# huttered40/capital

Measured on AMD Instinct MI355X. Metric: TFLOP/s (whole node) Cholesky n=65536, algorithmic n^3/3, recursive cholinv factor(), inputs resident in HBM, higher is better.
Workload: dtype f64

## Files before the change

### capital_amd/capi.py

```python
import ctypes as C
import os

import numpy as np
import torch

_HERE = os.path.dirname(os.path.abspath(__file__))
LIB_PATH = os.environ.get("CAPITAL_HIP_LIB", os.path.join(_HERE, "libcapital_hip.so"))

NOTRANS, TRANS = 0, 1
LEFT, RIGHT = 0, 1
LOWER, UPPER = 0, 1
NONUNIT, UNIT = 0, 1
RECT, UPPERTRI, LOWERTRI = 0, 1, 2

_i64, _dbl, _int, _vp = C.c_int64, C.c_double, C.c_int, C.c_void_p

_SIGS = {
    "capi_dgemm": [_int, _int, _i64, _i64, _i64, _dbl, _vp, _i64, _vp, _i64, _dbl, _vp, _i64],
    "capi_dsyrk": [_int, _int, _i64, _i64, _dbl, _vp, _i64, _dbl, _vp, _i64],
    "capi_dgemmt": [_int, _int, _int, _i64, _i64, _dbl, _vp, _i64, _vp, _i64, _dbl, _vp, _i64],
    "capi_dsyrk_panel32": [_i64, _i64, _dbl, _vp, _dbl, _vp, _i64],
    "capi_dtrmm_right_panel32": [_i64, _i64, _dbl, _vp, _i64, _vp, _i64, _vp, _i64],
    "capi_dtrmm": [_int, _int, _int, _int, _i64, _i64, _dbl, _vp, _i64, _vp, _i64],
    "capi_dtrmm_oop": [_int, _int, _int, _int, _i64, _i64, _dbl, _vp, _i64, _vp, _i64, _vp, _i64],
    "capi_dtrmm_acc": [_int, _int, _int, _int, _i64, _i64, _dbl, _vp, _i64, _vp, _i64, _dbl, _vp, _i64],
    "capi_dtrsm": [_int, _int, _int, _int, _i64, _i64, _dbl, _vp, _i64, _vp, _i64],
    "capi_dpotrf": [_int, _i64, _vp, _i64],
    "capi_dtrtri": [_int, _int, _i64, _vp, _i64],
    "capi_dpotrf_trtri": [_i64, _vp, _i64, _vp, _i64],
    "capi_dgram_equilibrate_shift": [_i64, _vp, _i64, _i64, _dbl, _vp, _vp],
    "capi_dtri_rescale": [_i64, _vp, _i64, _vp, _i64, _vp, _vp],
    "capi_dgemtn_ts": [_i64, _i64, _i64, _dbl, _vp, _i64, _vp, _i64, _dbl, _vp, _i64],
    "capi_dresid_ts": [_i64, _i64, _i64, _vp, _i64, _vp, _i64, _vp, _i64, _vp, _i64, _vp],
    "capi_dtrmm_thin": [_int, _int, _i64, _i64, _i64, _dbl, _vp, _i64, _i64, _vp, _i64, _dbl, _vp, _i64],
    "capi_get_info": [C.POINTER(_int)],
    "capi_reset_info": [],
    "capi_serialize": [_int, _int, _vp, _i64, _i64, _vp, _i64, _i64] + [_i64] * 8,
    "capi_serialize_shape": [_int, _int, _int, _vp, _i64, _i64, _vp, _i64, _i64] + [_i64] * 8,
    "capi_dlacpy": [_int, _i64, _i64, _vp, _i64, _vp, _i64],
    "capi_dgeadd": [_int, _i64, _i64, _dbl, _vp, _i64, _dbl, _vp, _i64],
    "capi_dtrizero": [_int, _i64, _vp, _i64],
    "capi_daxpby": [_i64, _dbl, _vp, _vp],
    "capi_remove_triangle": [C.c_char, _vp, _i64, _i64, _i64, _i64, _i64],
    "capi_block_to_cyclic": [_vp, _vp, _i64, _i64, _i64],
    "capi_block_to_cyclic_full": [_vp, _vp, _i64, _i64, _i64],
    "capi_cyclic_to_block": [_vp, _vp, _i64, _i64, _i64],
    "capi_block_to_cyclic_tri": [_vp, _vp, _i64, _i64],
# ... 161 lines not shown
```

### capital_amd/csrc/gemm_f64.hip

```cpp
#include "capi_internal.h"
#include "gemm_plan.h"
#include <type_traits>

extern "C" int capi_internal_copy2d(capi_handle_t h, int64_t m, int64_t n, const double* A, int64_t lda, double* B, int64_t ldb);

typedef double d4_t __attribute__((ext_vector_type(4)));
typedef double d2_t __attribute__((ext_vector_type(2)));

namespace {

constexpr int NTHREADS = 256;
using gemm_plan::BK, gemm_plan::SK;
template <int TS> struct tile_cfg {
  static constexpr int TILE_LDS = TS * SK;
  static constexpr int STAGE_LDS = 2 * TILE_LDS;
  static constexpr int NQ = TS / 32;
  static constexpr int SUB = TS / 32;
};
constexpr int GROUP_M = 8;
template <int TS> __device__ __forceinline__ int rc_r(int tid, int q) { return 16 * ((tid >> 6) * (TS / 64) + (q >> 1)) + 2 * (tid & 7); }
__device__ __forceinline__ int rc_k(int tid, int q) { return 8 * (q & 1) + ((tid >> 3) & 7); }

struct GemmArgs {
  const double* A;
// ... 4 lines not shown
  double alpha, beta;
  int out_uplo;
  int tri_side;
  int tri_eff_upper;
  int tri_unit;
  int a_vec, b_vec;
  int splitk, k_per_split;
  int k_rotate;
  double* slab;
  int64_t slab_ld, slab_stride;
  int tiles_m, tiles_n, ntiles;
  int batch;
  int64_t sa, sb, sc;
  int tail_base, tail_tm, tail_tn;
  int ts;
  int no_skip;
  int share_ab;
  int tri_dense;
  int tri_koff;
  int tri_block;
  int pid_base;
  int order;
  int a_tiled, c_tiled;
  unsigned long long* stamp;
};

__device__ __forceinline__ void stamp_begin(const GemmArgs& p) {
  if (p.stamp && threadIdx.x == 0) atomicMin(p.stamp, (unsigned long long)wall_clock64());
}
__device__ __forceinline__ void stamp_end(const GemmArgs& p) {
  if (p.stamp && threadIdx.x == 0) atomicMin(p.stamp + 1, ~(unsigned long long)wall_clock64());
}

template <int TS, bool KC>
__device__ __forceinline__ void panel_load(const double* __restrict__ X, int64_t ld, int r0, int R, int k0, int kend,
                                           int tid, bool vec_ok, d2_t (&v)[TS / 32]) {
  constexpr int NQ = TS / 32;
  if (KC) {
    const int kp = tid & 7, rb = tid >> 3;
    const int k = k0 + 2 * kp;
#pragma unroll
    for (int q = 0; q < NQ; ++q) {
      const int r = r0 + rb + 32 * q;
      d2_t val = {0.0, 0.0};
      if (r < R) {
        const double* p = X + (int64_t)r * ld + k;
// ... 349 lines not shown
      fa += (int64_t)(t - t_in) * ksa;
      fb += (int64_t)(t - t_in) * ksb;
    }
  }

  auto element_ok = [&](int i, int j) {
    bool ok = (i < p.M) && (j < p.N);
    if (p.out_uplo == CAPI_UPPER) ok = ok && (i <= j);
    if (p.out_uplo == CAPI_LOWER) ok = ok && (i >= j);
    return ok;
  };
  if (p.splitk > 1) {
#pragma unroll
    for (int a = 0; a < SUB; ++a) {
      const int i = i0 + wm * (TS / 2) + a * 16 + r16;
#pragma unroll
      for (int b = 0; b < SUB; ++b)
#pragma unroll
        for (int reg = 0; reg < 4; ++reg) {
          const int j = j0 + wn * (TS / 2) + b * 16 + g + 4 * reg;
          if (element_ok(i, j)) p.slab[(int64_t)z * p.slab_stride + i + (int64_t)j * p.slab_ld] = acc[a][b][reg];
        }
    }
  } else if (p.beta == 0.0) {
#pragma unroll
    for (int a = 0; a < SUB; ++a) {
      const int i = i0 + wm * (TS / 2) + a * 16 + r16;
#pragma unroll
      for (int b = 0; b < SUB; ++b)
#pragma unroll
        for (int reg = 0; reg < 4; ++reg) {
          const int j = j0 + wn * (TS / 2) + b * 16 + g + 4 * reg;
          if (element_ok(i, j)) p.C[i + (int64_t)j * p.ldc] = p.alpha * acc[a][b][reg];
        }
    }
  } else {
#pragma unroll
    for (int a = 0; a < SUB; ++a) {
      const int i = i0 + wm * (TS / 2) + a * 16 + r16;
      double old[SUB][4];
#pragma unroll
      for (int b = 0; b < SUB; ++b)
#pragma unroll
        for (int reg = 0; reg < 4; ++reg) {
          const int j = j0 + wn * (TS / 2) + b * 16 + g + 4 * reg;
          const bool ok = element_ok(i, j);
// ... 154 lines not shown
        panel_store<TS, AK>(Na, tid, ra);
        panel_store<TS, BKC>(Na + TILE_LDS, tid, rb);
      }
      par ^= 1;
      __syncthreads();
    };
    auto fast_run = [&](int tc) -> int {
      if (asc) return tc < tb0 ? max(0, min(tb0, ntk) - 1 - tc) : (tc >= tb1 ? max(0, ntk - 1 - tc) : 0);
      return tc >= tb1 ? tc - tb1 : (tc < tb0 ? tc : 0);
    };
    while (t >= 0 && t < ntk) {
      const int nf = fast_run(t);
      fa = fa0 + (int64_t)t * ksa;
      fb = fb0 + (int64_t)t * ksb;
      for (int q = 0; q < nf; ++q, t += dir) iterate(t, t + dir, std::true_type{});
      while (t >= 0 && t < ntk) {
        const int tn = t + dir;
        iterate(t, (tn >= 0 && tn < ntk) ? tn : -1, std::false_type{});
        t = tn;
        if (t >= 0 && t < ntk && fast_run(t) > 0) break;
      }
    }

#pragma unroll
    for (int a = 0; a < SUB; ++a) {
      const int i = i0 + wm * (TS / 2) + a * 16 + r16;
#pragma unroll
      for (int c = 0; c < SUB; ++c)
#pragma unroll
        for (int reg = 0; reg < 4; ++reg) {
          const int j = j0 + wn * (TS / 2) + c * 16 + g + 4 * reg;
          p.C[i + (int64_t)j * p.ldc] = p.alpha * acc[a][c][reg];
        }
    }
  }
  stamp_end(p);
}

__global__ void splitk_reduce_kernel(const double* __restrict__ slab, int64_t slab_ld, int64_t slab_stride, int splitk,
                                     double* __restrict__ C, int64_t ldc, int M, int N, double alpha, double beta, int out_uplo) {
  const int i = blockIdx.x * blockDim.x + threadIdx.x;
  if (i >= M) return;
  for (int j = blockIdx.y; j < N; j += gridDim.y) {
    if (out_uplo == CAPI_UPPER && i > j) continue;
    if (out_uplo == CAPI_LOWER && i < j) continue;
    double s = 0.0;
// ... 490 lines not shown
}

__global__ __launch_bounds__(TSK_THREADS, 1) void trmm_right_ts32_kernel(const GemmArgs p) {
  extern __shared__ __attribute__((aligned(16))) double lds[];
  switch (__builtin_amdgcn_readfirstlane(threadIdx.x >> 6)) {
    case 0: trmm_ts32_body<0>(p, lds); break;
    case 1: trmm_ts32_body<1>(p, lds); break;
    case 2: trmm_ts32_body<2>(p, lds); break;
    case 3: trmm_ts32_body<3>(p, lds); break;
    case 4: trmm_ts32_body<4>(p, lds); break;
    case 5: trmm_ts32_body<5>(p, lds); break;
    case 6: trmm_ts32_body<6>(p, lds); break;
    default: trmm_ts32_body<7>(p, lds); break;
  }
}

template <int TS>
gemm_kernel_t pick_kernel(bool ak, bool bkc) {
  return ak ? (bkc ? dgemm_tile_kernel<TS, true, true> : dgemm_tile_kernel<TS, true, false>)
            : (bkc ? dgemm_tile_kernel<TS, false, true> : dgemm_tile_kernel<TS, false, false>);
}

struct GemmEnv {
  bool debug;
  int no_skip;
  gemm_plan::Overrides ov;
};
const GemmEnv& gemm_env() {
  static const GemmEnv e = [] {
    const char* fts = getenv("CAPI_FORCE_TS");
    const char* fsm = getenv("CAPI_SMALL");
    return GemmEnv{getenv("CAPI_DEBUG_GEMM") != nullptr, getenv("CAPI_NO_SKIP") ? 1 : 0, {fts ? atoi(fts) : 0, fsm ? (atoi(fsm) != 0) : -1}};
  }();
  return e;
}

int launch_recorded(capi_handle_t h, gemm_kernel_t k, int64_t grid, size_t lds_bytes, GemmArgs q, double share, int variant) {
  capi_handle_s::prof_rec* rec = nullptr;
  if (h->prof_on) {
    if (h->prof_n == h->prof_cap) {
      const int ncap = h->prof_cap ? h->prof_cap * 2 : 1024;
      auto* np_ = (capi_handle_s::prof_rec*)realloc(h->prof, sizeof(capi_handle_s::prof_rec) * ncap);
      if (!np_) return CAPI_ENOMEM;
      for (int i = h->prof_cap; i < ncap; ++i) { np_[i].e0 = nullptr; np_[i].e1 = nullptr; }
      h->prof = np_;
      h->prof_cap = ncap;
    }
    rec = &h->prof[h->prof_n++];
    if (!rec->e0) { CAPI_HIP_CHECK(h, hipEventCreate(&rec->e0)); CAPI_HIP_CHECK(h, hipEventCreate(&rec->e1)); }
    rec->flops = q.out_uplo >= 0 ? (double)q.N * ((double)q.N + 1.0) * (double)q.K
                 : (q.tri_side >= 0 ? (q.tri_block ? (double)q.M * (double)q.N * (2.0 * (double)q.tri_koff + (double)q.N) : (double)q.M * (double)q.N * (double)q.K)
                                    : 2.0 * (double)q.M * (double)q.N * (double)q.K);
    rec->flops *= share;
    rec->variant = variant;
    rec->m = q.M; rec->n = q.N; rec->k = q.K; rec->kind = q.out_uplo >= 0 ? 1 : (q.tri_side >= 0 ? 2 : 0);
// ... 12 lines not shown
    hipLaunchKernelGGL(splitk_reduce_wide_kernel, dim3((unsigned)cdiv(p.M, 64), (unsigned)p.N), dim3(256), 0, h->stream, p.slab, p.slab_ld,
                       p.slab_stride, p.splitk, p.C, p.ldc, p.M, p.N, p.alpha, p.beta, p.out_uplo);
  else
    hipLaunchKernelGGL(splitk_reduce_kernel, dim3((unsigned)cdiv(p.M, 256), (unsigned)(p.N < 65535 ? p.N : 65535)), dim3(256), 0, h->stream,
                       p.slab, p.slab_ld, p.slab_stride, p.splitk, p.C, p.ldc, p.M, p.N, p.alpha, p.beta, p.out_uplo);
  CAPI_HIP_CHECK(h, hipGetLastError());
  return CAPI_OK;
}

int launch_gemm(capi_handle_t h, bool ak, bool bkc, GemmArgs& p, bool ws_for_slab) {
  using gemm_plan::Path;
  const GemmEnv& env = gemm_env();
  gemm_plan::Product d;
  d.M = p.M; d.N = p.N; d.K = p.K; d.out_uplo = p.out_uplo;
  d.tri_side = p.tri_side; d.tri_eff_upper = p.tri_eff_upper; d.tri_dense = p.tri_dense; d.tri_block = p.tri_block; d.tri_koff = p.tri_koff;
  d.alpha_zero = p.alpha == 0.0; d.beta = p.beta; d.batch = p.batch; d.ak = ak; d.bkc = bkc;
  d.a_is_b = p.A == p.B; d.same_ld = p.lda == p.ldb;
  d.a_vec = (((uintptr_t)p.A & 15) == 0) && ((p.lda & 1) == 0);
  d.b_vec = (((uintptr_t)p.B & 15) == 0) && ((p.ldb & 1) == 0);
  d.a_tiled = p.a_tiled; d.c_tiled = p.c_tiled; d.ws_for_slab = ws_for_slab;
  const gemm_plan::Device dev{h->num_cu, h->cu_of[h->cur]};
  const gemm_plan::Modes modes{h->rounds_mode, h->pair_mode, h->pair_rounds, h->pair_rounds_min};
  const gemm_plan::Plan pl = gemm_plan::plan(d, dev, modes, env.ov);
  if (env.debug) {
    char line[2048];
    gemm_plan::format(line, sizeof(line), d, dev, modes, env.ov, pl);
    fprintf(stderr, "[capi gemm] %s\n", line);
  }
  hipStream_t s = h->stream;
  if (pl.path == Path::none) return CAPI_OK;
  CAPI_REQUIRE(h, pl.path != Path::refused, "panel32 operand reached a kernel that does not read it");
  if (pl.path == Path::scale) {
    dim3 grid((unsigned)cdiv(p.M, 256), (unsigned)(p.N < 65535 ? p.N : 65535));
    hipLaunchKernelGGL(scale_kernel, grid, dim3(256), 0, s, p.C, p.ldc, p.M, p.N, p.beta, p.out_uplo);
    CAPI_HIP_CHECK(h, hipGetLastError());
    return CAPI_OK;
  }
  if (pl.path == Path::trmm_ts32) {
    p.a_vec = d.a_vec;
    p.splitk = 1;
    CAPI_RAISE_LDS_LIMIT(h, CAPI_ATTR_TRMM_TS32, trmm_right_ts32_kernel, pl.lds_bytes);
    hipLaunchKernelGGL(trmm_right_ts32_kernel, dim3((unsigned)pl.blocks), dim3(TSK_THREADS), pl.lds_bytes, s, p);
    CAPI_HIP_CHECK(h, hipGetLastError());
    return CAPI_OK;
  }
  if (pl.path == Path::gram_blocks) {
    for (int J = 0; J < pl.tiles_n; ++J)
      for (int I = 0; I <= J; ++I) {
        GemmArgs q = p;
        q.A = p.A + (int64_t)I * TSK_W * p.lda;
// ... 124 lines not shown
  CAPI_REQUIRE(h, n >= 0 && k >= 0 && n < (1LL << 31) && k < (1LL << 31), "dims");
  if (n == 0) return CAPI_OK;
  CAPI_REQUIRE(h, C && ldc >= n, "C/ldc");
  if (k > 0) {
    CAPI_REQUIRE(h, A && B, "null operand");
    CAPI_REQUIRE(h, lda >= (transA ? k : n) && ldb >= (transB ? n : k), "lda/ldb");
  }
  GemmArgs p{};
  p.A = A; p.B = B; p.C = C; p.lda = lda; p.ldb = ldb; p.ldc = ldc;
  p.M = (int)n; p.N = (int)n; p.K = (int)k; p.alpha = alpha; p.beta = beta;
  p.out_uplo = uplo; p.tri_side = -1;
  return launch_gemm(h, transA == CAPI_TRANS, transB == CAPI_NOTRANS, p, true);
}

int capi_dsyrk(capi_handle_t h, int uplo, int trans, int64_t n, int64_t k, double alpha,
               const double* A, int64_t lda, double beta, double* C, int64_t ldc) {
  CAPI_REQUIRE(h, h, "null handle");
  CAPI_REQUIRE(h, ok01(trans), "transpose code");
  return capi_dgemmt(h, uplo, trans, trans == CAPI_TRANS ? CAPI_NOTRANS : CAPI_TRANS, n, k, alpha, A, lda, A, lda, beta, C, ldc);
}

static int trmm_launch(capi_handle_t h, int side, int uplo, int trans, int diag, int64_t m, int64_t n, double alpha,
                       const double* T, int64_t ldt, const double* B, int64_t ldb, double beta, double* C, int64_t ldc,
                       bool ws_free = true) {
  CAPI_REQUIRE(h, h, "null handle");
  CAPI_REQUIRE(h, ok01(side) && ok01(uplo) && ok01(trans) && ok01(diag), "enum code");
  CAPI_REQUIRE(h, m >= 0 && n >= 0 && m < (1LL << 31) && n < (1LL << 31), "dims");
  if (m == 0 || n == 0) return CAPI_OK;
  const int64_t nt = side == CAPI_LEFT ? m : n;
  CAPI_REQUIRE(h, T && B && C && ldt >= nt && ldb >= m && ldc >= m, "operands");
  CAPI_REQUIRE(h, (const double*)C != B, "out-of-place trmm: C aliases B");
  GemmArgs p{};
  p.C = C; p.ldc = ldc; p.M = (int)m; p.N = (int)n; p.K = (int)nt; p.alpha = alpha; p.beta = beta;
  p.out_uplo = -1;
  p.tri_side = side;
  p.tri_eff_upper = ((uplo == CAPI_UPPER) != (trans == CAPI_TRANS));
  p.tri_unit = diag == CAPI_UNIT;
  if (side == CAPI_RIGHT && diag == CAPI_NONUNIT && n >= 512 && n <= 4096 && m >= 64 * n) {
    void* w;
    int rc = capi_ws3_get(h, sizeof(double) * (size_t)n * (size_t)n, &w);
    if (rc != CAPI_OK) return rc;
    CAPI_HIP_CHECK(h, hipMemsetAsync(w, 0, sizeof(double) * (size_t)n * (size_t)n, h->stream));
    rc = capi_dlacpy(h, uplo == CAPI_UPPER ? 1 : 2, n, n, T, ldt, (double*)w, n);
    if (rc != CAPI_OK) return rc;
    T = (const double*)w;
    ldt = n;
    p.tri_dense = 1;
    const bool eff_upper = (uplo == CAPI_UPPER) != (trans == CAPI_TRANS);
    if (eff_upper && n % 256 == 0) {
      for (int64_t J = 0; J < n / 256; ++J) {
        GemmArgs q = p;
        q.N = 256;
        q.K = (int)(256 * (J + 1));
        q.tri_koff = (int)(256 * J);
        q.tri_block = 1;
        q.C = C + 256 * J * ldc;
        q.A = B; q.lda = ldb;
        q.B = trans == CAPI_NOTRANS ? T + 256 * J * ldt : T + 256 * J;
        q.ldb = ldt;
        int rc2 = launch_gemm(h, false, trans == CAPI_NOTRANS, q, ws_free);
        if (rc2 != CAPI_OK) return rc2;
      }
      return CAPI_OK;
    }
  }
  if (side == CAPI_LEFT) {
    p.A = T; p.lda = ldt; p.B = B; p.ldb = ldb;
    return launch_gemm(h, trans == CAPI_TRANS, true, p, ws_free);
  } else {
    p.A = B; p.lda = ldb; p.B = T; p.ldb = ldt;
    return launch_gemm(h, false, trans == CAPI_NOTRANS, p, ws_free);
  }
}

__attribute__((visibility("hidden"))) int capi_internal_trmm_oop_batched(capi_handle_t h, int side, int uplo, int trans, int diag,
                                                                           int64_t m, int64_t n, double alpha, const double* T,
                                                                           int64_t ldt, int64_t st, const double* B, int64_t ldb,
                                                                           int64_t sb_, double* C, int64_t ldc, int64_t sc_, int batch) {
  CAPI_REQUIRE(h, h && m >= 0 && n >= 0 && m < (1LL << 31) && n < (1LL << 31) && batch >= 0, "dims");
  const bool small_ok = m <= 512 && n <= 512 && gemm_env().ov.force_small < 0;
  const bool aligned = ((st | sb_ | sc_) & 1) == 0;
  if (batch > 1 && small_ok && aligned) {
    const int64_t nt = side == CAPI_LEFT ? m : n;
    GemmArgs p{};
    p.C = C; p.ldc = ldc; p.M = (int)m; p.N = (int)n; p.K = (int)nt; p.alpha = alpha; p.beta = 0.0;
    p.out_uplo = -1; p.tri_side = side;
    p.tri_eff_upper = ((uplo == CAPI_UPPER) != (trans == CAPI_TRANS));
    p.tri_unit = diag == CAPI_UNIT;
    p.batch = batch;
    if (side == CAPI_LEFT) { p.A = T; p.lda = ldt; p.sa = st; p.B = B; p.ldb = ldb; p.sb = sb_; p.sc = sc_; return launch_gemm(h, trans == CAPI_TRANS, true, p, true); }
    p.A = B; p.lda = ldb; p.sa = sb_; p.B = T; p.ldb = ldt; p.sb = st; p.sc = sc_;
    return launch_gemm(h, false, trans == CAPI_NOTRANS, p, true);
  }
  for (int b = 0; b < batch; ++b) {
    int rc = capi_dtrmm_oop(h, side, uplo, trans, diag, m, n, alpha, T + b * st, ldt, B + b * sb_, ldb, C + b * sc_, ldc);
    if (rc != CAPI_OK) return rc;
  }
  return CAPI_OK;
}

int capi_dtrmm_oop(capi_handle_t h, int side, int uplo, int trans, int diag, int64_t m, int64_t n, double alpha,
                   const double* T, int64_t ldt, const double* B, int64_t ldb, double* C, int64_t ldc) {
  return trmm_launch(h, side, uplo, trans, diag, m, n, alpha, T, ldt, B, ldb, 0.0, C, ldc);
}

int capi_dtrmm_acc(capi_handle_t h, int side, int uplo, int trans, int diag, int64_t m, int64_t n, double alpha,
                   const double* T, int64_t ldt, const double* B, int64_t ldb, double beta, double* C, int64_t ldc) {
  return trmm_launch(h, side, uplo, trans, diag, m, n, alpha, T, ldt, B, ldb, beta, C, ldc);
}

int capi_dtrmm(capi_handle_t h, int side, int uplo, int trans, int diag, int64_t m, int64_t n, double alpha,
               const double* T, int64_t ldt, double* B, int64_t ldb) {
  CAPI_REQUIRE(h, h, "null handle");
  if (m <= 0 || n <= 0) return m < 0 || n < 0 ? CAPI_EINVAL : CAPI_OK;
  void* ws;
  int rc = capi_ws_get(h, sizeof(double) * (size_t)m * (size_t)n, &ws);
  if (rc != CAPI_OK) return rc;
  rc = trmm_launch(h, side, uplo, trans, diag, m, n, alpha, T, ldt, B, ldb, 0.0, (double*)ws, m, false);
  if (rc != CAPI_OK) return rc;
  return capi_internal_copy2d(h, m, n, (const double*)ws, m, B, ldb);
}

int capi_dsyrk_panel32(capi_handle_t h, int64_t n, int64_t k, double alpha, const double* A32, double beta, double* C, int64_t ldc) {
  CAPI_REQUIRE(h, h, "null handle");
  CAPI_REQUIRE(h, n == TSK_W && k > 0 && k % 32 == 0 && k >= 64 * n && k < (1LL << 31), "panel32 Gram matrix: n == 256, k a multiple of 32, k >= 64 n");
  CAPI_REQUIRE(h, A32 && C && ldc >= n && (((uintptr_t)A32 & 15) == 0), "operands");
// ... 129 lines not shown
```

### capital_amd/csrc/gemm_plan.h

```cpp
#ifndef CAPITAL_GEMM_PLAN_H_
#define CAPITAL_GEMM_PLAN_H_

#include <cstddef>
#include <cstdint>
#include <cstdio>

#include "capital_hip.h"

namespace gemm_plan {

constexpr int BK = 16;
constexpr int SK = BK + 2;
constexpr int ST = 32, SKC = 256, SQK = 64, SLD = ST + 2;
constexpr int TSK_W = 256;

inline int64_t cdiv(int64_t a, int64_t b) { return (a + b - 1) / b; }

struct Product {
  int M = 0, N = 0, K = 0;
  int out_uplo = -1;
  int tri_side = -1;
  int tri_eff_upper = 0, tri_dense = 0, tri_block = 0, tri_koff = 0;
  bool alpha_zero = false;
  double beta = 0.0;
// ... 170 lines not shown
    if (r.ntiles >= 2 * per_round && rem > 0 && rem <= (3 * per_round) / 4) r.tail128 = rem;
  }
  const int ntiles_all = r.ntiles;
  r.ntiles -= r.tail128;
  r.blocks = (int64_t)r.ntiles * r.splitk;
  r.per_launch = use_rounds ? per_round : r.blocks;
  r.lds_bytes = sizeof(double) * 2 * 2 * (size_t)r.ts * SK;
  r.variant = vi + (r.ts == 128 ? 0 : 4);
  r.share_den = (double)ntiles_all * r.splitk;
  const int ntri = p.tri_side == CAPI_LEFT ? r.tiles_m : r.tiles_n, nfree = p.tri_side == CAPI_LEFT ? r.tiles_n : r.tiles_m;
  const int64_t wgs = (int64_t)(ntri / 2) * nfree;
  if (mode.pair_mode && tri && !p.tri_dense && !p.tri_block && p.tri_koff == 0 && r.ts == 128 && r.splitk == 1 && p.beta == 0.0 &&
      p.batch <= 1 && p.M % 128 == 0 && p.N % 128 == 0 && p.K % 128 == 0 && p.a_vec && p.b_vec && (ntri & 1) == 0 && wgs % per_round == 0 &&
      (mode.pair_mode > 1 || wgs <= 4 * per_round || (mode.pair_rounds && p.K >= mode.pair_rounds_min))) {
    r.path = Path::pair;
    r.blocks = wgs;
    r.per_launch = mode.pair_rounds && wgs > per_round && p.K >= mode.pair_rounds_min ? per_round : wgs;
    r.variant = vi + 16;
    r.share_den = (double)wgs;
  }
  return r;
}

inline int format(char* buf, size_t n, const Product& p, const Device& d, const Modes& m, const Overrides& o, const Plan& r) {
  static const char* const reduce_names[] = {"none", "narrow", "wide"};
  return snprintf(buf, n,
                  "M=%d N=%d K=%d out_uplo=%d tri_side=%d tri_eff_upper=%d tri_dense=%d tri_block=%d tri_koff=%d alpha_zero=%d beta=%.17g "
                  "batch=%d ak=%d bkc=%d a_is_b=%d same_ld=%d a_vec=%d b_vec=%d a_tiled=%d c_tiled=%d ws_for_slab=%d num_cu=%d stream_cu=%d "
                  "rounds_mode=%d pair_mode=%d pair_rounds=%d pair_rounds_min=%d force_ts=%d force_small=%d -> path=%s ts=%d splitk=%d "
                  "k_per_split=%d k_rotate=%d order=%d share_ab=%d slab_stride=%lld tiles_m=%d tiles_n=%d ntiles=%d blocks=%lld "
                  "per_launch=%lld launches=%lld grid_y=%d tail128=%d reduce=%s lds=%zu variant=%d share_den=%.17g est_us=%.1f small_est_us=%.1f",
                  p.M, p.N, p.K, p.out_uplo, p.tri_side, p.tri_eff_upper, p.tri_dense, p.tri_block, p.tri_koff, (int)p.alpha_zero, p.beta,
                  p.batch, (int)p.ak, (int)p.bkc, (int)p.a_is_b, (int)p.same_ld, (int)p.a_vec, (int)p.b_vec, (int)p.a_tiled, (int)p.c_tiled,
                  (int)p.ws_for_slab, d.num_cu, d.stream_cu, m.rounds_mode, m.pair_mode, m.pair_rounds, m.pair_rounds_min, o.force_ts,
                  o.force_small, path_name(r.path), r.ts, r.splitk, r.k_per_split, r.k_rotate, r.order, r.share_ab, (long long)r.slab_stride,
                  r.tiles_m, r.tiles_n, r.ntiles, (long long)r.blocks, (long long)r.per_launch, (long long)r.launches(), r.grid_y, r.tail128,
                  reduce_names[(int)r.reduce], r.lds_bytes, r.variant, r.share_den, r.est_us, r.small_est_us);
}

}

#endif
```

### capital_amd/src/alg/cholesky/cholinv/cholinv.h

```cpp
#ifndef CAPITAL_CHOLESKY_CHOLINV_H_
#define CAPITAL_CHOLESKY_CHOLINV_H_

#include "./../../alg.h"
#include "./../../matmult/summa/summa.h"
#include "./policy.h"

#pragma weak capi_dtrmm_thin
#pragma weak capi_dresid_ts

namespace cholesky {

template <class SerializePolicy = policy::cholinv::Serialize, class IntermediatesPolicy = policy::cholinv::SaveIntermediates,
          class BaseCasePolicy = policy::cholinv::NoReplication>
class cholinv : public SerializePolicy, public IntermediatesPolicy, public BaseCasePolicy {
public:
  using SP = SerializePolicy;
  using IP = IntermediatesPolicy;
  using BP = BaseCasePolicy;

  template <typename ScalarT, typename DimensionT>
  class info {
  public:
    using ScalarType = ScalarT;
    using DimensionType = DimensionT;
    using alg_type = cholinv<SerializePolicy, IntermediatesPolicy, BaseCasePolicy>;
    using SP = SerializePolicy;
    using IP = IntermediatesPolicy;
    using BP = BaseCasePolicy;
    info(const info& p) : complete_inv(p.complete_inv), split(p.split), bc_mult_dim(p.bc_mult_dim), dir(p.dir) {}
    info(info&& p) : complete_inv(p.complete_inv), split(p.split), bc_mult_dim(p.bc_mult_dim), dir(p.dir) {}
    info(DimensionType complete_inv, DimensionType split, DimensionType bc_mult_dim, char dir)
        : complete_inv(complete_inv), split(split), bc_mult_dim(bc_mult_dim), dir(dir) {}
    const DimensionType complete_inv, split, bc_mult_dim;
    const char dir;
    matrix<ScalarType, DimensionType, typename SerializePolicy::structure> R, Rinv;
    matrix<ScalarType, DimensionType, rect> Rfull, Rinvfull;
    matmult::arena work;
    DimensionType localDimension = 0, globalDimension = 0, trueLocalDimension = 0, trueGlobalDimension = 0, bcDimension = 0;
    int64_t num_base_cases = 0, num_levels = 0;
    bool solve_with_trsm = false;
    int potrf_info = 0;
    bool zeroed = false;
    const double* input = nullptr;
    DimensionType early_split = 0;
    DimensionType input_lead = 0;
    int la_depth = 0;
    bool factored = false, factored_trsm = false;
    DimensionType top_split = 0;
    matrix<ScalarType, DimensionType, rect> X, SolveW1, SolveW2, SolveRho, SolveD, SolveNorm2;
    std::vector<double> solve_residual_norms;
  };

  template <typename MatrixType, typename ArgType, typename CommType>
  static void factor(const MatrixType& A, ArgType& args, CommType&& CommInfo) {
    CRITTER_START(CI::factor);
    using U = typename ArgType::DimensionType;
    static_assert(std::is_same<typename MatrixType::StructureType, rect>::value, "cholinv::factor takes a rect-structured input block");
    if (!(args.split > 0) || args.dir != 'U') throw std::invalid_argument("cholinv: split > 0 and dir == 'U' required (cholinv.hpp:9)");
    if (CommInfo.d > 1 && CommInfo.d % CommInfo.c) throw std::invalid_argument("cholinv: c must divide d (or d == 1)");
    args.factored = false;
    args.factored_trsm = args.solve_with_trsm;
    args.top_split = 0;
    if (args.solve_with_trsm) { factor_trsm(A, args, CommInfo); args.factored = true; CRITTER_STOP(CI::factor); return; }
    const U localDimension = A.num_rows_local(), globalDimension = A.num_rows_global();
    CAPITAL_CHECK(capi_stream_select(capital::handle(), 0));
    CAPITAL_CHECK(capi_reset_info(capital::handle()));
    args.potrf_info = 0;
    args.R._register_(A.num_columns_global(), A.num_rows_global(), CommInfo.d, CommInfo.d);
    args.Rinv._register_(A.num_columns_global(), A.num_rows_global(), CommInfo.d, CommInfo.d);
    constexpr bool packed = !std::is_same<typename SP::structure, rect>::value;
    if (packed) {
      args.Rfull._register_(A.num_columns_global(), A.num_rows_global(), CommInfo.d, CommInfo.d);
      args.Rinvfull._register_(A.num_columns_global(), A.num_rows_global(), CommInfo.d, CommInfo.d);
    }
    double* R = packed ? args.Rfull.data() : (double*)args.R.data();
    double* Ri = packed ? args.Rinvfull.data() : (double*)args.Rinv.data();
    const U ld = localDimension;
    if (!args.zeroed) {
      capital::dev_zero(R, ld * ld);
      capital::dev_zero(Ri, ld * ld);
      args.zeroed = true;
    }
    U bcDimLocal = (U)(CommInfo.c * CommInfo.d);
    U bcMult = args.bc_mult_dim;
    if (bcMult < 0) { bcMult = -bcMult; for (U i = 0; i < bcMult; ++i) bcDimLocal *= 2; } else { for (U i = 0; i < bcMult; ++i) bcDimLocal /= 2; }
    bcDimLocal = std::max<U>(1, bcDimLocal);
    bcDimLocal = std::min<U>(localDimension, bcDimLocal);
    bcDimLocal = localDimension / bcDimLocal;
    args.localDimension = args.trueLocalDimension = localDimension;
    args.globalDimension = args.trueGlobalDimension = globalDimension;
    args.bcDimension = (U)CommInfo.d * bcDimLocal;
    args.num_base_cases = args.num_levels = 0;

    const U h1 = localDimension >> args.split;
    args.input = A.data();
    args.early_split = 0;
    const bool will_split = !(((localDimension * (U)CommInfo.d) <= args.bcDimension) || (h1 < args.split));
    args.input_lead = 0;
    args.top_split = will_split ? h1 : 0;
    if (will_split && h1 > 0 && h1 < ld) {
      capi_handle_t hh = capital::handle();
      U lead = h1;
      if (args.split == 1 && CommInfo.d == 1 && CommInfo.c == 1) while (lead >= 8192 && lead % 2 == 0 && (lead >> 1) * (U)CommInfo.d > args.bcDimension) lead >>= 1;
      CAPITAL_CHECK(capi_dlacpy(hh, 1, lead, lead, A.data(), ld, R, ld));
      CAPITAL_CHECK(capi_event_record(hh, EV_INPUT_HEAD));
      CAPITAL_CHECK(capi_stream_select(hh, 1));
      CAPITAL_CHECK(capi_event_wait(hh, EV_INPUT_HEAD));
      if (lead < h1) {
        CAPITAL_CHECK(capi_dlacpy(hh, 0, lead, h1 - lead, A.data() + (int64_t)lead * ld, ld, R + (int64_t)lead * ld, ld));
        CAPITAL_CHECK(capi_dlacpy(hh, 1, h1 - lead, h1 - lead, A.data() + lead + (int64_t)lead * ld, ld, R + lead + (int64_t)lead * ld, ld));
        CAPITAL_CHECK(capi_event_record(hh, EV_INPUT_MID));
        args.input_lead = lead;
      }
      CAPITAL_CHECK(capi_dlacpy(hh, 0, h1, ld - h1, A.data() + (int64_t)h1 * ld, ld, R + (int64_t)h1 * ld, ld));
      CAPITAL_CHECK(capi_dlacpy(hh, 1, ld - h1, ld - h1, A.data() + h1 + (int64_t)h1 * ld, ld, R + h1 + (int64_t)h1 * ld, ld));
      CAPITAL_CHECK(capi_event_record(hh, EV_INPUT_REST));
      CAPITAL_CHECK(capi_stream_select(hh, 0));
      args.early_split = h1;
    } else {
      CAPITAL_CHECK(capi_dlacpy(capital::handle(), 1, ld, ld, A.data(), ld, R, ld));
    }


    const bool single = (CommInfo.d == 1 && CommInfo.c == 1);
    capital::launch_rounds_scope rounds(true);
    const U h = localDimension - (localDimension >> args.split);
    const U agg = args.bcDimension;
    int64_t need = single ? (int64_t)h * h + (int64_t)h * h / 3 + 1024 : (int64_t)(CommInfo.d == 1 ? 8 : 12) * h * h + 4 * (int64_t)agg * agg + 4096;
    args.work.reserve(need);

    args.la_depth = 0;
    invoke(args, CommInfo, R, Ri, ld, (U)0, localDimension, globalDimension);

    if (packed) {
      const U e = args.early_split;
      if (e > 0) {
        pack_block(args, CAPI_UPPERTRI, R, (double*)args.R.data(), ld, e, ld, e, ld);
        pack_block(args, CAPI_UPPERTRI, Ri, (double*)args.Rinv.data(), ld, e, ld, e, ld);
        if (args.complete_inv) pack_block(args, CAPI_RECT, Ri, (double*)args.Rinv.data(), ld, e, ld, 0, e);
        CAPITAL_CHECK(capi_event_wait(capital::handle(), EV_EARLY_PACK));
      } else {
        serialize<uppertri, uppertri>::invoke(args.Rfull, args.R, 0, ld, 0, ld, 0, ld, 0, ld);
        serialize<uppertri, uppertri>::invoke(args.Rinvfull, args.Rinv, 0, ld, 0, ld, 0, ld, 0, ld);
      }
    }
    if (!IP::keep_arena) {
      capital::sync();
      args.work.release();
      if (packed) { args.Rfull._destroy_(); args.Rinvfull._destroy_(); args.zeroed = false; }
    }
    CRITTER_STOP(CI::factor);
    CAPITAL_CHECK(capi_get_info(capital::handle(), &args.potrf_info));
    const int failed = capital::ranks_with_nonzero(CommInfo.world, args.potrf_info);
    if (failed != 0)
      throw std::domain_error("cholinv::factor: the matrix is not positive definite (" +
                              (args.potrf_info != 0 ? "non-positive pivot " + std::to_string(args.potrf_info) + " of a diagonal block"
                                                    : std::string("reported by ") + std::to_string(failed) + " other rank(s) of the grid") +
// ... 273 lines not shown
      CRITTER_STOP(CI::factor_diag);
      return;
    }
    ++args.num_levels;
    const U split2 = localDim - split1;
    const bool single = (t.d == 1 && t.c == 1);
    matmult::arena& ws = args.work;
    view R11i{Ri + start + start * ld, ld, split1, split1};
    view A12{R + start + (start + split1) * ld, ld, split1, split2};
    view A22{R + (start + split1) + (start + split1) * ld, ld, split2, split2};
    view R22i{Ri + (start + split1) + (start + split1) * ld, ld, split2, split2};
    view I12{Ri + start + (start + split1) * ld, ld, split1, split2};

    invoke(args, t, R, Ri, ld, start, split1, globalDim >> 1);
    if (wait_ev >= 0) CAPITAL_CHECK(capi_event_wait(h, wait_ev));
    if (start == 0 && args.input_lead > 0 && split1 == args.input_lead) CAPITAL_CHECK(capi_event_wait(h, EV_INPUT_MID));

    const bool top = (localDim == args.localDimension) && args.early_split == split1;
    if (top) CAPITAL_CHECK(capi_event_wait(h, EV_INPUT_REST));
    CRITTER_START(CI::trsm);
    int child_wait = -1;
    bool copy_deferred = false;
    const int64_t mark = ws.top;
    {
      view W{ws.take((int64_t)split1 * split2), split1, split1, split2};
      if (single) {
        CAPITAL_CHECK(capi_dtrmm_oop(h, CAPI_LEFT, CAPI_UPPER, CAPI_TRANS, CAPI_NONUNIT, split1, split2, 1.0, R11i.p, ld, A12.p, ld, W.p, W.ld));
      } else {
        view Tx{ws.take((int64_t)split1 * split1), split1, split1, split1};
        const int64_t np = matmult::summa::tri_count(split1);
        if ((t.x == t.y && !t.multipath) || !matmult::summa::packed_comm()) {
          CAPITAL_CHECK(capi_dlacpy(h, 0, split1, split1, R11i.p, ld, Tx.p, Tx.ld));
          util::transpose_raw(Tx.p, Tx.count(), ws.take(Tx.count()), t, matmult::summa::relay_space(t, Tx.count(), ws));
        } else if (t.x == t.y) {
          CAPITAL_CHECK(capi_dlacpy(h, 0, split1, split1, R11i.p, ld, Tx.p, Tx.ld));
          util::transpose_raw(nullptr, np, nullptr, t, matmult::summa::relay_space(t, np, ws));
        } else {
          double* pk = ws.take(np);
          matmult::summa::pack_tri(R11i, CAPI_UPPER, pk);
          util::transpose_raw(pk, np, ws.take(np), t, matmult::summa::relay_space(t, np, ws));
          matmult::summa::unpack_tri(pk, CAPI_UPPER, Tx);
        }
        matmult::summa::trmm(t, CAPI_LEFT, CAPI_UPPER, CAPI_TRANS, CAPI_NONUNIT, 1.0, Tx, A12, W, ws);
      }
      const U lead = split2 >> args.split;
      const bool a22_splits = !(((split2 * (U)t.d) <= args.bcDimension) || (lead < args.split));
      const bool la = single && a22_splits && lead > 0 && lookahead_min() >= 0 && (int64_t)split2 >= lookahead_min() && args.la_depth < lookahead_depth();
      const bool pack_now = top && !std::is_same<typename SP::structure, rect>::value;
      const bool copy_later = la && pack_now && !getenv("CAPITAL_PACK_AT_ONCE");
      if (!copy_later) CAPITAL_CHECK(capi_dlacpy(h, 0, split1, split2, W.p, W.ld, A12.p, ld));
      copy_deferred = copy_later;
      CRITTER_STOP(CI::trsm);
      auto early_pack = [&](int after_ev) {
        CAPITAL_CHECK(capi_stream_select(h, 1));
        CAPITAL_CHECK(capi_event_wait(h, after_ev));
        if (copy_later) CAPITAL_CHECK(capi_dlacpy(h, 0, split1, split2, W.p, W.ld, A12.p, ld));
        pack_block(args, CAPI_UPPERTRI, R, (double*)args.R.data(), ld, (U)0, split1, (U)0, split1);
        pack_block(args, CAPI_RECT, R, (double*)args.R.data(), ld, split1, ld, (U)0, split1);
        pack_block(args, CAPI_UPPERTRI, Ri, (double*)args.Rinv.data(), ld, (U)0, split1, (U)0, split1);
        CAPITAL_CHECK(capi_event_record(h, EV_EARLY_PACK));
        CAPITAL_CHECK(capi_stream_select(h, 0));
      };
      bool packed_early = false;

      CRITTER_START(CI::tmu);
      if (la) {
        const int depth = args.la_depth;
        const U rest = split2 - lead;
        double* Wr = W.p + (int64_t)lead * W.ld;
        CAPITAL_CHECK(capi_dgemmt(h, CAPI_UPPER, CAPI_TRANS, CAPI_NOTRANS, lead, split1, -1.0, W.p, W.ld, W.p, W.ld, 1.0, A22.p, ld));
        CAPITAL_CHECK(capi_event_record(h, EV_LA_LEAD + depth));
        CAPITAL_CHECK(capi_stream_select(h, LA_STREAM0 + depth));
        CAPITAL_CHECK(capi_event_wait(h, EV_LA_LEAD + depth));
// ... 10 lines not shown
      } else {
        view Wx{ws.take(W.count()), split1, split1, split2};
        capital::dev_copy(Wx.p, W.p, W.count());
        util::transpose_raw(Wx.p, Wx.count(), ws.take(Wx.count()), t, matmult::summa::relay_space(t, Wx.count(), ws));
        matmult::summa::syrk(t, CAPI_UPPER, CAPI_TRANS, -1.0, W, Wx, 1.0, A22, ws);
      }
      if (pack_now && !packed_early) {
        CAPITAL_CHECK(capi_event_record(h, EV_TOP_R12));
        early_pack(EV_TOP_R12);
      }
      if (child_wait < 0) ws.top = mark;
      CRITTER_STOP(CI::tmu);
    }

    invoke(args, t, R, Ri, ld, start + split1, split2, split2 * (U)t.d, child_wait);
    if (child_wait >= 0) { --args.la_depth; ws.top = mark; }

    CRITTER_START(CI::tmu);
    if (!(!args.complete_inv && (globalDim == args.trueGlobalDimension))) {
      if (copy_deferred) CAPITAL_CHECK(capi_event_wait(h, EV_EARLY_PACK));
      const int64_t mark = ws.top;
      view W2{ws.take((int64_t)split1 * split2), split1, split1, split2};
      matmult::summa::trmm(t, CAPI_LEFT, CAPI_UPPER, CAPI_NOTRANS, CAPI_NONUNIT, 1.0, R11i, A12, W2, ws);
      if (single) {
        matmult::summa::trmm(t, CAPI_RIGHT, CAPI_UPPER, CAPI_NOTRANS, CAPI_NONUNIT, -1.0, R22i, W2, I12, ws);
      } else {
        view W3{ws.take(W2.count()), split1, split1, split2};
        matmult::summa::trmm(t, CAPI_RIGHT, CAPI_UPPER, CAPI_NOTRANS, CAPI_NONUNIT, -1.0, R22i, W2, W3, ws);
        CAPITAL_CHECK(capi_dlacpy(h, 0, split1, split2, W3.p, W3.ld, I12.p, ld));
      }
      ws.top = mark;
    }
    CRITTER_STOP(CI::tmu);
  }

  template <typename ArgType, typename CommType, typename U>
  static void base_case(ArgType& args, CommType&& t, double* R, double* Ri, U ld, U start, U localDim) {
    capi_handle_t h = capital::handle();
    ++args.num_base_cases;
    double* Rb = R + start + start * ld;
    double* Ib = Ri + start + start * ld;
    if (t.d == 1) {
      CAPITAL_CHECK(capi_dpotrf_trtri(h, localDim, Rb, ld, Ib, ld));
      return;
    }
    const int64_t d = (int64_t)t.d, L = (int64_t)localDim, agg = L * d;
    const int64_t span = ((start + localDim) != args.trueLocalDimension) ? agg : agg - (args.trueLocalDimension * d - args.trueGlobalDimension);
    constexpr bool packed_msg = !std::is_same<typename SP::structure, rect>::value;
    const int64_t piece = packed_msg ? L * (L + 1) / 2 : L * L;
    auto pack_piece = [&](const double* blk, double* dst) {
      if (packed_msg) CAPITAL_CHECK(capi_serialize_shape(h, CAPI_UPPERTRI, CAPI_RECT, CAPI_UPPERTRI, blk, ld, ld, dst, L, L, 0, L, 0, L, 0, L, 0, L));
      else CAPITAL_CHECK(capi_dlacpy(h, 0, L, L, blk, ld, dst, L));
    };
    auto unpack_piece = [&](const double* src, double* blk) {
      if (packed_msg) CAPITAL_CHECK(capi_serialize_shape(h, CAPI_UPPERTRI, CAPI_UPPERTRI, CAPI_RECT, src, L, L, blk, ld, ld, 0, L, 0, L, 0, L, 0, L));
      else CAPITAL_CHECK(capi_dlacpy(h, 0, L, L, src, L, blk, ld));
    };
    auto to_cyclic = [&](const double* blocked, double* cyc) {
      if (packed_msg) CAPITAL_CHECK(capi_block_to_cyclic_tri(h, blocked, cyc, L, d));
      else util::block_to_cyclic_rect(blocked, cyc, L, L, d);
    };
    auto to_blocked = [&](double* blocked, const double* cyc) {
      if (packed_msg) CAPITAL_CHECK(capi_cyclic_to_block_tri(h, blocked, cyc, L, d));
      else util::cyclic_to_block_rect(blocked, cyc, L, L, d);
    };
    matmult::arena& ws = args.work;
// ... 78 lines not shown
```

### include/capital_hip.h

```cpp
#ifndef CAPITAL_HIP_H_
#define CAPITAL_HIP_H_

#include <stddef.h>
#include <stdint.h>

#ifdef __cplusplus
extern "C" {
#endif

typedef struct capi_handle_s* capi_handle_t;
typedef struct capi_comm_s*   capi_comm_t;

enum capi_status {
  CAPI_OK = 0,
  CAPI_EINVAL = -1,
  CAPI_EHIP = -2,
  CAPI_ENOMEM = -3,
  CAPI_ECOMM = -4,
  CAPI_ENOTSPD = -5
};
enum { CAPI_NOTRANS = 0, CAPI_TRANS = 1 };
enum { CAPI_LEFT = 0, CAPI_RIGHT = 1 };
enum { CAPI_LOWER = 0, CAPI_UPPER = 1 };
enum { CAPI_NONUNIT = 0, CAPI_UNIT = 1 };
// ... 8 lines not shown
const char* capi_last_error(capi_handle_t h);
int  capi_malloc(capi_handle_t h, void** dptr, size_t bytes);
int  capi_free(capi_handle_t h, void* dptr);
int  capi_memset_async(capi_handle_t h, void* dptr, int value, size_t bytes);
int  capi_memcpy_h2d(capi_handle_t h, void* dst, const void* src, size_t bytes);
int  capi_memcpy_d2h(capi_handle_t h, void* dst, const void* src, size_t bytes);
int  capi_memcpy_d2d_async(capi_handle_t h, void* dst, const void* src, size_t bytes);
int  capi_sync(capi_handle_t h);
int  capi_reserve_workspace(capi_handle_t h, size_t bytes);
int  capi_trim_workspaces(capi_handle_t h);
int  capi_set_launch_rounds(capi_handle_t h, int on, int* was);
int  capi_reserve_cus(capi_handle_t h, int reserve);

int capi_dgemm(capi_handle_t h, int transA, int transB, int64_t m, int64_t n, int64_t k, double alpha,
               const double* A, int64_t lda, const double* B, int64_t ldb, double beta, double* C, int64_t ldc);
int capi_dsyrk(capi_handle_t h, int uplo, int trans, int64_t n, int64_t k, double alpha,
               const double* A, int64_t lda, double beta, double* C, int64_t ldc);
int capi_dgemmt(capi_handle_t h, int uplo, int transA, int transB, int64_t n, int64_t k, double alpha,
                const double* A, int64_t lda, const double* B, int64_t ldb, double beta, double* C, int64_t ldc);
int capi_dtrmm(capi_handle_t h, int side, int uplo, int trans, int diag, int64_t m, int64_t n, double alpha,
               const double* T, int64_t ldt, double* B, int64_t ldb);
int capi_dtrmm_oop(capi_handle_t h, int side, int uplo, int trans, int diag, int64_t m, int64_t n, double alpha,
                   const double* T, int64_t ldt, const double* B, int64_t ldb, double* C, int64_t ldc);
int capi_dtrmm_acc(capi_handle_t h, int side, int uplo, int trans, int diag, int64_t m, int64_t n, double alpha,
                   const double* T, int64_t ldt, const double* B, int64_t ldb, double beta, double* C, int64_t ldc);
int capi_dtrsm(capi_handle_t h, int side, int uplo, int trans, int diag, int64_t m, int64_t n, double alpha,
               const double* T, int64_t ldt, double* B, int64_t ldb);

int capi_dsyrk_panel32(capi_handle_t h, int64_t n, int64_t k, double alpha, const double* A32, double beta, double* C, int64_t ldc);
int capi_dtrmm_right_panel32(capi_handle_t h, int64_t m, int64_t n, double alpha, const double* T, int64_t ldt,
                             const double* B, int64_t ldb, double* C, int64_t ldc);
int capi_dpotrf(capi_handle_t h, int uplo, int64_t n, double* A, int64_t lda);
int capi_dtrtri(capi_handle_t h, int uplo, int diag, int64_t n, double* A, int64_t lda);
int capi_dpotrf_trtri(capi_handle_t h, int64_t n, double* A, int64_t lda, double* Rinv, int64_t ldi);
int capi_get_info(capi_handle_t h, int* info);
int capi_dgram_equilibrate_shift(capi_handle_t h, int64_t n, double* G, int64_t ldg, int64_t m_global, double shift_scale,
                                 double* dscale, double* rec);
int capi_dtri_rescale(capi_handle_t h, int64_t n, double* R, int64_t ldr, double* Rinv, int64_t ldi, const double* dscale, double* rec);
enum { CAPI_TS_MAX_RHS = 32 };
int capi_dgemtn_ts(capi_handle_t h, int64_t m, int64_t n, int64_t r, double alpha, const double* A, int64_t lda, const double* B, int64_t ldb,
                   double beta, double* C, int64_t ldc);
int capi_dresid_ts(capi_handle_t h, int64_t m, int64_t n, int64_t r, const double* A, int64_t lda, const double* X, int64_t ldx,
                   const double* B, int64_t ldb, double* Rout, int64_t ldr, double* colnorm2);
int capi_dtrmm_thin(capi_handle_t h, int shape, int trans, int64_t m, int64_t n, int64_t r, double alpha,
                    const double* T, int64_t ldt, int64_t col0, const double* B, int64_t ldb, double beta, double* C, int64_t ldc);
int capi_dgeqrf(capi_handle_t h, int64_t m, int64_t n, double* A, int64_t lda, double* tau);
// ... 66 lines not shown
```

Baseline: 55.56.

## Write TRMM results directly into packed triangular output from GEMM epilogue

Adds a second-destination epilogue to the f64 GEMM kernel so a TRMM can store its block both to the dense buffer and to the packed upper-triangular output in one pass. Cholinv uses it for the R12 and Rinv12 blocks and packs diagonal leaf blocks right away, which removes the separate packing passes at the end. At the top level the input's A12 is read directly as the TRMM source, which skips one dlacpy and shrinks the workspace reservation. The cost is extra scattered stores in the epilogue, plus a fallback to explicit packing when the GEMM plan refuses the second destination.

```diff
diff --git a/capital_amd/capi.py b/capital_amd/capi.py
--- a/capital_amd/capi.py
+++ b/capital_amd/capi.py
@@ -23,6 +23,7 @@
     "capi_dtrmm_right_panel32": [_i64, _i64, _dbl, _vp, _i64, _vp, _i64, _vp, _i64],
     "capi_dtrmm": [_int, _int, _int, _int, _i64, _i64, _dbl, _vp, _i64, _vp, _i64],
     "capi_dtrmm_oop": [_int, _int, _int, _int, _i64, _i64, _dbl, _vp, _i64, _vp, _i64, _vp, _i64],
+    "capi_dtrmm_oop_packed": [_int, _int, _int, _int, _i64, _i64, _dbl, _vp, _i64, _vp, _i64, _vp, _i64, _vp, _i64, _i64, C.POINTER(_int)],
     "capi_dtrmm_acc": [_int, _int, _int, _int, _i64, _i64, _dbl, _vp, _i64, _vp, _i64, _dbl, _vp, _i64],
     "capi_dtrsm": [_int, _int, _int, _int, _i64, _i64, _dbl, _vp, _i64, _vp, _i64],
     "capi_dpotrf": [_int, _i64, _vp, _i64],
diff --git a/capital_amd/csrc/gemm_f64.hip b/capital_amd/csrc/gemm_f64.hip
--- a/capital_amd/csrc/gemm_f64.hip
+++ b/capital_amd/csrc/gemm_f64.hip
@@ -50,6 +50,8 @@
   int pid_base;
   int order;
   int a_tiled, c_tiled;
+  double* C2;
+  int64_t c2_row0, c2_col0;
   unsigned long long* stamp;
 };
 
@@ -445,6 +447,23 @@
           if (element_ok(i, j)) p.slab[(int64_t)z * p.slab_stride + i + (int64_t)j * p.slab_ld] = acc[a][b][reg];
         }
     }
+  } else if (p.beta == 0.0 && p.C2) {
+#pragma unroll
+    for (int a = 0; a < SUB; ++a) {
+      const int i = i0 + wm * (TS / 2) + a * 16 + r16;
+#pragma unroll
+      for (int b = 0; b < SUB; ++b)
+#pragma unroll
+        for (int reg = 0; reg < 4; ++reg) {
+          const int j = j0 + wn * (TS / 2) + b * 16 + g + 4 * reg;
+          const int64_t J = p.c2_col0 + j;
+          if (element_ok(i, j)) {
+            const double v = p.alpha * acc[a][b][reg];
+            p.C[i + (int64_t)j * p.ldc] = v;
+            p.C2[((J * (J + 1)) >> 1) + p.c2_row0 + i] = v;
+          }
+        }
+    }
   } else if (p.beta == 0.0) {
 #pragma unroll
     for (int a = 0; a < SUB; ++a) {
@@ -645,6 +664,23 @@
       }
     }
 
+    if (p.C2) {
+#pragma unroll
+      for (int a = 0; a < SUB; ++a) {
+        const int i = i0 + wm * (TS / 2) + a * 16 + r16;
+#pragma unroll
+        for (int c = 0; c < SUB; ++c)
+#pragma unroll
+          for (int reg = 0; reg < 4; ++reg) {
+            const int j = j0 + wn * (TS / 2) + c * 16 + g + 4 * reg;
+            const int64_t J = p.c2_col0 + j;
+            const double v = p.alpha * acc[a][c][reg];
+            p.C[i + (int64_t)j * p.ldc] = v;
+            p.C2[((J * (J + 1)) >> 1) + p.c2_row0 + i] = v;
+          }
+      }
+      continue;
+    }
 #pragma unroll
     for (int a = 0; a < SUB; ++a) {
       const int i = i0 + wm * (TS / 2) + a * 16 + r16;
@@ -1181,7 +1217,6 @@
 }
 
 struct GemmEnv {
-  bool debug;
   int no_skip;
   gemm_plan::Overrides ov;
 };
@@ -1189,7 +1224,7 @@
   static const GemmEnv e = [] {
     const char* fts = getenv("CAPI_FORCE_TS");
     const char* fsm = getenv("CAPI_SMALL");
-    return GemmEnv{getenv("CAPI_DEBUG_GEMM") != nullptr, getenv("CAPI_NO_SKIP") ? 1 : 0, {fts ? atoi(fts) : 0, fsm ? (atoi(fsm) != 0) : -1}};
+    return GemmEnv{getenv("CAPI_NO_SKIP") ? 1 : 0, {fts ? atoi(fts) : 0, fsm ? (atoi(fsm) != 0) : -1}};
   }();
   return e;
 }
@@ -1248,10 +1283,12 @@
   const gemm_plan::Device dev{h->num_cu, h->cu_of[h->cur]};
   const gemm_plan::Modes modes{h->rounds_mode, h->pair_mode, h->pair_rounds, h->pair_rounds_min};
   const gemm_plan::Plan pl = gemm_plan::plan(d, dev, modes, env.ov);
-  if (env.debug) {
+  const bool asked_c2 = p.C2 != nullptr;
+  if (asked_c2 && !gemm_plan::second_dest_ok(d, pl)) p.C2 = nullptr;
+  if (getenv("CAPI_DEBUG_GEMM")) {
     char line[2048];
     gemm_plan::format(line, sizeof(line), d, dev, modes, env.ov, pl);
-    fprintf(stderr, "[capi gemm] %s\n", line);
+    fprintf(stderr, "[capi gemm] %s second_dest=%s\n", line, !asked_c2 ? "none" : (p.C2 ? "stored" : "refused"));
   }
   hipStream_t s = h->stream;
   if (pl.path == Path::none) return CAPI_OK;
@@ -1422,7 +1459,8 @@
 
 static int trmm_launch(capi_handle_t h, int side, int uplo, int trans, int diag, int64_t m, int64_t n, double alpha,
                        const double* T, int64_t ldt, const double* B, int64_t ldb, double beta, double* C, int64_t ldc,
-                       bool ws_free = true) {
+                       bool ws_free = true, double* C2 = nullptr, int64_t row0 = 0, int64_t col0 = 0, int* stored = nullptr) {
+  if (stored) *stored = 0;
   CAPI_REQUIRE(h, h, "null handle");
   CAPI_REQUIRE(h, ok01(side) && ok01(uplo) && ok01(trans) && ok01(diag), "enum code");
   CAPI_REQUIRE(h, m >= 0 && n >= 0 && m < (1LL << 31) && n < (1LL << 31), "dims");
@@ -1464,13 +1502,17 @@
       return CAPI_OK;
     }
   }
+  p.C2 = C2; p.c2_row0 = row0; p.c2_col0 = col0;
+  int rc;
   if (side == CAPI_LEFT) {
     p.A = T; p.lda = ldt; p.B = B; p.ldb = ldb;
-    return launch_gemm(h, trans == CAPI_TRANS, true, p, ws_free);
+    rc = launch_gemm(h, trans == CAPI_TRANS, true, p, ws_free);
   } else {
     p.A = B; p.lda = ldb; p.B = T; p.ldb = ldt;
-    return launch_gemm(h, false, trans == CAPI_NOTRANS, p, ws_free);
-  }
+    rc = launch_gemm(h, false, trans == CAPI_NOTRANS, p, ws_free);
+  }
+  if (stored && rc == CAPI_OK) *stored = p.C2 != nullptr;
+  return rc;
 }
 
 __attribute__((visibility("hidden"))) int capi_internal_trmm_oop_batched(capi_handle_t h, int side, int uplo, int trans, int diag,
@@ -1502,6 +1544,16 @@
 int capi_dtrmm_oop(capi_handle_t h, int side, int uplo, int trans, int diag, int64_t m, int64_t n, double alpha,
                    const double* T, int64_t ldt, const double* B, int64_t ldb, double* C, int64_t ldc) {
   return trmm_launch(h, side, uplo, trans, diag, m, n, alpha, T, ldt, B, ldb, 0.0, C, ldc);
+}
+
+int capi_dtrmm_oop_packed(capi_handle_t h, int side, int uplo, int trans, int diag, int64_t m, int64_t n, double alpha,
+                          const double* T, int64_t ldt, const double* B, int64_t ldb, double* C, int64_t ldc,
+                          double* packed, int64_t row0, int64_t col0, int* stored) {
+  if (stored) *stored = 0;
+  CAPI_REQUIRE(h, h, "null handle");
+  CAPI_REQUIRE(h, packed && stored, "packed destination and its result flag expected");
+  CAPI_REQUIRE(h, row0 >= 0 && col0 >= 0 && m >= 0 && n >= 0 && row0 + m <= col0 + 1, "the block must lie wholly above the packed triangle's diagonal");
+  return trmm_launch(h, side, uplo, trans, diag, m, n, alpha, T, ldt, B, ldb, 0.0, C, ldc, true, packed, row0, col0, stored);
 }
 
 int capi_dtrmm_acc(capi_handle_t h, int side, int uplo, int trans, int diag, int64_t m, int64_t n, double alpha,
diff --git a/capital_amd/csrc/gemm_plan.h b/capital_amd/csrc/gemm_plan.h
--- a/capital_amd/csrc/gemm_plan.h
+++ b/capital_amd/csrc/gemm_plan.h
@@ -216,6 +216,11 @@
   return r;
 }
 
+inline bool second_dest_ok(const Product& p, const Plan& r) {
+  return (r.path == Path::tile || r.path == Path::pair) && r.splitk == 1 && p.beta == 0.0 && p.out_uplo < 0 && !p.tri_block && !p.tri_dense &&
+         p.batch <= 1 && !p.a_tiled && !p.c_tiled;
+}
+
 inline int format(char* buf, size_t n, const Product& p, const Device& d, const Modes& m, const Overrides& o, const Plan& r) {
   static const char* const reduce_names[] = {"none", "narrow", "wide"};
   return snprintf(buf, n,
diff --git a/capital_amd/src/alg/cholesky/cholinv/cholinv.h b/capital_amd/src/alg/cholesky/cholinv/cholinv.h
--- a/capital_amd/src/alg/cholesky/cholinv/cholinv.h
+++ b/capital_amd/src/alg/cholesky/cholinv/cholinv.h
@@ -7,6 +7,7 @@
 
 #pragma weak capi_dtrmm_thin
 #pragma weak capi_dresid_ts
+#pragma weak capi_dtrmm_oop_packed
 
 namespace cholesky {
 
@@ -44,6 +45,7 @@
     const double* input = nullptr;
     DimensionType early_split = 0;
     DimensionType input_lead = 0;
+    bool pack_direct = false;
     int la_depth = 0;
     bool factored = false, factored_trsm = false;
     DimensionType top_split = 0;
@@ -76,6 +78,7 @@
     double* R = packed ? args.Rfull.data() : (double*)args.R.data();
     double* Ri = packed ? args.Rinvfull.data() : (double*)args.Rinv.data();
     const U ld = localDimension;
+    args.pack_direct = packed && CommInfo.d == 1 && CommInfo.c == 1 && &capi_dtrmm_oop_packed && !getenv("CAPITAL_PACK_PASSES");
     if (!args.zeroed) {
       capital::dev_zero(R, ld * ld);
       capital::dev_zero(Ri, ld * ld);
@@ -112,7 +115,7 @@
         CAPITAL_CHECK(capi_event_record(hh, EV_INPUT_MID));
         args.input_lead = lead;
       }
-      CAPITAL_CHECK(capi_dlacpy(hh, 0, h1, ld - h1, A.data() + (int64_t)h1 * ld, ld, R + (int64_t)h1 * ld, ld));
+      if (!args.pack_direct) CAPITAL_CHECK(capi_dlacpy(hh, 0, h1, ld - h1, A.data() + (int64_t)h1 * ld, ld, R + (int64_t)h1 * ld, ld));
       CAPITAL_CHECK(capi_dlacpy(hh, 1, ld - h1, ld - h1, A.data() + h1 + (int64_t)h1 * ld, ld, R + h1 + (int64_t)h1 * ld, ld));
       CAPITAL_CHECK(capi_event_record(hh, EV_INPUT_REST));
       CAPITAL_CHECK(capi_stream_select(hh, 0));
@@ -126,13 +129,14 @@
     capital::launch_rounds_scope rounds(true);
     const U h = localDimension - (localDimension >> args.split);
     const U agg = args.bcDimension;
-    int64_t need = single ? (int64_t)h * h + (int64_t)h * h / 3 + 1024 : (int64_t)(CommInfo.d == 1 ? 8 : 12) * h * h + 4 * (int64_t)agg * agg + 4096;
+    const bool top_direct = args.pack_direct && args.early_split > 0;
+    int64_t need = single ? (top_direct && !args.complete_inv ? (int64_t)h * h / 4 : (int64_t)h * h) + (int64_t)h * h / 3 + 1024 : (int64_t)(CommInfo.d == 1 ? 8 : 12) * h * h + 4 * (int64_t)agg * agg + 4096;
     args.work.reserve(need);
 
     args.la_depth = 0;
     invoke(args, CommInfo, R, Ri, ld, (U)0, localDimension, globalDimension);
 
-    if (packed) {
+    if (packed && !args.pack_direct) {
       const U e = args.early_split;
       if (e > 0) {
         pack_block(args, CAPI_UPPERTRI, R, (double*)args.R.data(), ld, e, ld, e, ld);
@@ -452,9 +456,18 @@
     int child_wait = -1;
     bool copy_deferred = false;
     const int64_t mark = ws.top;
+    const bool direct = args.pack_direct;
+    const bool from_input = direct && top && args.input != nullptr;
     {
-      view W{ws.take((int64_t)split1 * split2), split1, split1, split2};
-      if (single) {
+      view W = from_input ? A12 : view{ws.take((int64_t)split1 * split2), split1, split1, split2};
+      if (direct) {
+        const double* src = from_input ? args.input + start + (int64_t)(start + split1) * ld : A12.p;
+        int stored = 0;
+        CAPITAL_CHECK(capi_dtrmm_oop_packed(h, CAPI_LEFT, CAPI_UPPER, CAPI_TRANS, CAPI_NONUNIT, split1, split2, 1.0, R11i.p, ld, src, ld, W.p, W.ld,
+                                            (double*)args.R.data(), start, start + split1, &stored));
+        if (!from_input) CAPITAL_CHECK(capi_dlacpy(h, 0, split1, split2, W.p, W.ld, A12.p, ld));
+        if (!stored) pack_block(args, CAPI_RECT, R, (double*)args.R.data(), ld, start + split1, start + localDim, start, start + split1);
+      } else if (single) {
         CAPITAL_CHECK(capi_dtrmm_oop(h, CAPI_LEFT, CAPI_UPPER, CAPI_TRANS, CAPI_NONUNIT, split1, split2, 1.0, R11i.p, ld, A12.p, ld, W.p, W.ld));
       } else {
         view Tx{ws.take((int64_t)split1 * split1), split1, split1, split1};
@@ -476,9 +489,9 @@
       const U lead = split2 >> args.split;
       const bool a22_splits = !(((split2 * (U)t.d) <= args.bcDimension) || (lead < args.split));
       const bool la = single && a22_splits && lead > 0 && lookahead_min() >= 0 && (int64_t)split2 >= lookahead_min() && args.la_depth < lookahead_depth();
-      const bool pack_now = top && !std::is_same<typename SP::structure, rect>::value;
+      const bool pack_now = top && !direct && !std::is_same<typename SP::structure, rect>::value;
       const bool copy_later = la && pack_now && !getenv("CAPITAL_PACK_AT_ONCE");
-      if (!copy_later) CAPITAL_CHECK(capi_dlacpy(h, 0, split1, split2, W.p, W.ld, A12.p, ld));
+      if (!copy_later && !direct) CAPITAL_CHECK(capi_dlacpy(h, 0, split1, split2, W.p, W.ld, A12.p, ld));
       copy_deferred = copy_later;
       CRITTER_STOP(CI::trsm);
       auto early_pack = [&](int after_ev) {
@@ -535,7 +548,12 @@
       const int64_t mark = ws.top;
       view W2{ws.take((int64_t)split1 * split2), split1, split1, split2};
       matmult::summa::trmm(t, CAPI_LEFT, CAPI_UPPER, CAPI_NOTRANS, CAPI_NONUNIT, 1.0, R11i, A12, W2, ws);
-      if (single) {
+      if (args.pack_direct) {
+        int stored = 0;
+        CAPITAL_CHECK(capi_dtrmm_oop_packed(h, CAPI_RIGHT, CAPI_UPPER, CAPI_NOTRANS, CAPI_NONUNIT, split1, split2, -1.0, R22i.p, ld, W2.p, W2.ld, I12.p, ld,
+                                            (double*)args.Rinv.data(), start, start + split1, &stored));
+        if (!stored) pack_block(args, CAPI_RECT, Ri, (double*)args.Rinv.data(), ld, start + split1, start + localDim, start, start + split1);
+      } else if (single) {
         matmult::summa::trmm(t, CAPI_RIGHT, CAPI_UPPER, CAPI_NOTRANS, CAPI_NONUNIT, -1.0, R22i, W2, I12, ws);
       } else {
         view W3{ws.take(W2.count()), split1, split1, split2};
@@ -555,6 +573,10 @@
     double* Ib = Ri + start + start * ld;
     if (t.d == 1) {
       CAPITAL_CHECK(capi_dpotrf_trtri(h, localDim, Rb, ld, Ib, ld));
+      if (args.pack_direct) {
+        pack_block(args, CAPI_UPPERTRI, R, (double*)args.R.data(), ld, start, start + localDim, start, start + localDim);
+        pack_block(args, CAPI_UPPERTRI, Ri, (double*)args.Rinv.data(), ld, start, start + localDim, start, start + localDim);
+      }
       return;
     }
     const int64_t d = (int64_t)t.d, L = (int64_t)localDim, agg = L * d;
diff --git a/include/capital_hip.h b/include/capital_hip.h
--- a/include/capital_hip.h
+++ b/include/capital_hip.h
@@ -54,6 +54,9 @@
                const double* T, int64_t ldt, double* B, int64_t ldb);
 int capi_dtrmm_oop(capi_handle_t h, int side, int uplo, int trans, int diag, int64_t m, int64_t n, double alpha,
                    const double* T, int64_t ldt, const double* B, int64_t ldb, double* C, int64_t ldc);
+int capi_dtrmm_oop_packed(capi_handle_t h, int side, int uplo, int trans, int diag, int64_t m, int64_t n, double alpha,
+                          const double* T, int64_t ldt, const double* B, int64_t ldb, double* C, int64_t ldc,
+                          double* packed, int64_t row0, int64_t col0, int* stored);
 int capi_dtrmm_acc(capi_handle_t h, int side, int uplo, int trans, int diag, int64_t m, int64_t n, double alpha,
                    const double* T, int64_t ldt, const double* B, int64_t ldb, double beta, double* C, int64_t ldc);
 int capi_dtrsm(capi_handle_t h, int side, int uplo, int trans, int diag, int64_t m, int64_t n, double alpha,
```

New measurement: 56.09 (median of 6 runs). About the same (+1.0%).
